# zhangganlin/GlORIE-SLAM

Measured on AMD Instinct MI355X. Metric: DSPO BA-update iters/sec + rendered rays/sec, 640x480 Replica keyframe graph, higher is better.
Workload: dtype f16 corr/ConvGRU, f32 Jacobians, f64 solve; render: f32 (decoder matmuls as 3-term f16 splits, f32 accumulate); 1 GPU; G8: 8 keyframes, 36 edges, 60x80 (640x480/8), BA itrs=2, DSPO stages alternating, context part of the GRU gates (one map per source keyframe) re-evaluated for all keyframes every 12 steps; multiview_filter.thresh = 0.25 (reference ships 0.01, configs/mono_point_slam.yaml:75: with untrained weights 0.01 rejects > 80 % of every frame and no depth_scale step would reach stage 2); render: 524k-point c; edges_local=36, edges_total=36, hw=4800, keyframes=8, parallelism=single GPU

## Files before the change

glorie_slam_amd/csrc/ba.hip:

```cpp
#include <hip/hip_runtime.h>
#include <stdint.h>
#include <math.h>
#include "common.hiph"
#include "se3.hiph"
#include "ba_common.hiph"

namespace glorie {

__device__ __forceinline__ void block_inclusive_scan(int* a, int n) {
  const int tid = threadIdx.x;
  for (int off = 1; off < n; off <<= 1) {
    int tmp[4];
#pragma unroll
    for (int q = 0; q < 4; ++q) {
      const int f = tid + q * 1024;
      tmp[q] = (f < n) ? a[f] + (f >= off ? a[f - off] : 0) : 0;
    }
    __syncthreads();
#pragma unroll
    for (int q = 0; q < 4; ++q) {
      const int f = tid + q * 1024;
      if (f < n) a[f] = tmp[q];
    }
    __syncthreads();
  }
}

__global__ __launch_bounds__(1024) void ba_prepare_kernel(BaWork wk, const int64_t* __restrict__ ii,
                                                          int B, int N, int M, int t0, int t1) {
  if (ba_skipped(wk)) return;
  extern __shared__ int sm[];
  int* cnt = sm;
  int* scan = sm + B;
  int* slot = sm + 2 * B;
  int* eii = sm + 3 * B;
  const int tid = threadIdx.x;
  if (tid == 0 && wk.gate_hits) atomicAdd(wk.gate_hits, 1);
  for (int f = tid; f < B; f += 1024) cnt[f] = 0;
  if (tid < 4) wk.status[tid] = 0;
  __syncthreads();
  for (int n = tid; n < N; n += 1024) {
    const int f = (int)ii[n];
    eii[n] = f;
    if (f >= 0 && f < B) atomicAdd(&cnt[f], 1);
  }
  __syncthreads();
  for (int f = tid; f < B; f += 1024) scan[f] = (cnt[f] > 0 || (f >= t0 && f < t1)) ? 1 : 0;
  __syncthreads();
  block_inclusive_scan(scan, B);
  const int Mdev = B > 0 ? scan[B - 1] : 0;
  for (int f = tid; f < B; f += 1024) {
    const int present = (cnt[f] > 0 || (f >= t0 && f < t1)) ? 1 : 0;
    const int sl = present ? scan[f] - 1 : -1;
    slot[f] = sl;
    wk.slot_of_frame[f] = sl;
    if (sl >= 0 && sl < M) wk.kx[sl] = f;
  }
  if (tid == 0) {
    wk.status[1] = Mdev;
    if (Mdev != M) atomicOr(&wk.status[0], BA_ST_M_MISMATCH);
  }
  __syncthreads();
  if (Mdev != M) return;
  for (int sl = tid; sl < M; sl += 1024) scan[sl] = 0;
  __syncthreads();
  for (int f = tid; f < B; f += 1024)
    if (slot[f] >= 0) scan[slot[f]] = cnt[f];
  __syncthreads();
  block_inclusive_scan(scan, M);
  for (int sl = tid; sl <= M; sl += 1024) wk.csr_ptr[sl] = (sl == 0) ? 0 : scan[sl - 1];
  for (int f = tid; f < B; f += 1024) {
    const int sl = slot[f];
    if (sl < 0 || cnt[f] == 0) continue;
    int o = (sl == 0) ? 0 : scan[sl - 1];
    for (int n = 0; n < N; ++n)
      if (eii[n] == f) wk.csr_edge[o++] = n;
  }
}

struct PixJ {
  float Ju[6], Jv[6];
  float Jzu, Jzv;
  float ru, rv;
  float wu, wv;
};

__device__ __forceinline__ void pixel_terms(const Pose g, float fx, float fy, float cx, float cy,
                                            float u, float v, float disp, float tu, float tv,
                                            float wgt_u, float wgt_v, PixJ& o) {
  float Xi[4], Xj[4];
  Xi[0] = (u - cx) / fx;
  Xi[1] = (v - cy) / fy;
  Xi[2] = 1.0f;
  Xi[3] = disp;
  se3_act(g, Xi, Xj);
  const float x = Xj[0], y = Xj[1], hh = Xj[3];
  const bool near = Xj[2] < 0.25f;
  const float d = near ? 0.0f : 1.0f / Xj[2];
  const float d2 = d * d;
  o.wu = near ? 0.0f : 0.001f * wgt_u;
  o.wv = near ? 0.0f : 0.001f * wgt_v;
  o.ru = tu - (fx * d * x + cx);
  o.rv = tv - (fy * d * y + cy);
  o.Ju[0] = fx * (hh * d);
  o.Ju[1] = fx * 0.0f;
  o.Ju[2] = fx * (-x * hh * d2);
  o.Ju[3] = fx * (-x * y * d2);
  o.Ju[4] = fx * (1.0f + x * x * d2);
  o.Ju[5] = fx * (-y * d);
  o.Jzu = fx * (g.t.x * d - g.t.z * (x * d2));
  o.Jv[0] = fy * 0.0f;
  o.Jv[1] = fy * (hh * d);
  o.Jv[2] = fy * (-y * hh * d2);
  o.Jv[3] = fy * (-1.0f - y * y * d2);
  o.Jv[4] = fy * (x * y * d2);
  o.Jv[5] = fy * (x * d);
  o.Jzv = fy * (g.t.y * d - g.t.z * (y * d2));
}

__device__ __forceinline__ void edge_adjoint(const Pose g, float L[36]) {
#pragma unroll
  for (int m = 0; m < 6; ++m) {
    float X[6] = {0, 0, 0, 0, 0, 0}, Y[6];
    X[m] = 1.0f;
    se3_adjT(g, X, Y);
#pragma unroll
    for (int r = 0; r < 6; ++r) L[r * 6 + m] = Y[r];
  }
}

// ... 548 lines not shown
      hr[q] = Bj[ok[q] ? o_ar[q] - 1 : 0];
      hc[q] = Bj[ok[q] ? o_ac[q] - 1 : 0];
      cur[q] = Bj[ok[q] ? o_w[q] : 0];
      if (!inr) ar[q] = 0.0;
      if (!inc) ac[q] = 0.0;
    }
    const bool rok = j + 1 + rhs_dc < n, rin = rok && rhs_dc < bw;
    double ra = Bj[rin ? o_rc : 0];
    const double rh = Bj[rok ? o_rc - 1 : 0];
    const double ru = u[rok ? j + 1 + rhs_dc : 0];
    const double u0 = u[j], u1h = u[j + 1];
    if (!rin) ra = 0.0;
    const double ri0 = rcp_f64(d0);
    const double d1 = h11 - a1 * ri0 * a1;
    if ((!(d0 > 0.0) || !(d1 > 0.0)) && tid == 0) *fail = 1;
    const double ri1 = rcp_f64(d1);
    if (tid == 0) { rinv[j] = ri0; rinv[j + 1] = ri1; }
#pragma unroll
    for (int q = 0; q < NQ; ++q) {
      if (pend_on[q]) B[(j - 2) * S + o_w[q]] = pend[q];
      pend_on[q] = false;
      if (!ok[q]) continue;
      double v = cur[q] - ar[q] * ri0 * ac[q];
      if (e_dc[q] > 0) {
        const double br = hr[q] - ar[q] * ri0 * a1, bc = hc[q] - ac[q] * ri0 * a1;
        v -= br * ri1 * bc;
        B[j * S + o_w[q]] = v;
      } else {
        pend[q] = v;
        pend_on[q] = true;
      }
    }
    if (rok) {
      double v = ru - u0 * ri0 * ra;
      if (rhs_dc > 0) {
        const double u1 = u1h - u0 * ri0 * a1, bc = rh - ra * ri0 * a1;
        v -= u1 * ri1 * bc;
      }
      u[j + 1 + rhs_dc] = v;
    }
    __syncthreads();
  }
#pragma unroll
  for (int q = 0; q < NQ; ++q)
    if (pend_on[q]) B[(j - 2) * S + o_w[q]] = pend[q];
  if (j < n) {
    const double d = B[j * S];
    if (!(d > 0.0) && tid == 0) *fail = 1;
    if (tid == 0) rinv[j] = rcp_f64(d);
  }
  __syncthreads();
}

__global__ __launch_bounds__(kBandThreads) void ba_solve_band_kernel(BaWork wk, int n, float lm, float ep,
                                                                    int lds_doubles, int force_bw, int from_acc) {
  if (ba_skipped(wk)) return;
  extern __shared__ double bsm[];
  __shared__ int fail, bw_s;
  const int tid = threadIdx.x;
  const double* A = wk.Hd;
  if (tid == 0) {
    fail = (wk.status[0] & (BA_ST_M_MISMATCH | BA_ST_NONFINITE)) ? 1 : 0;
    bw_s = force_bw >= 0 ? force_bw : wk.status[3] >> 1;
  }
  __syncthreads();
  const int bw = bw_s;
  const int S = bw + 1;
  if (bw >= 64 || (size_t)n * S + 2 * (size_t)n > (size_t)lds_doubles) {
    return;
  }
  double* B = bsm;
  double* u = B + (size_t)n * S;
  double* rinv = u + n;
  for (int base = tid; base < n * S; base += kBandThreads * 8) {
    double v[8];
    int rr[8], kk[8];
#pragma unroll
    for (int q = 0; q < 8; ++q) {
      const int idx = base + q * kBandThreads;
      const int r = idx / S, k = S - 1 - (idx - r * S);
      rr[q] = r; kk[q] = k;
      v[q] = (idx < n * S && k <= r) ? (from_acc ? acc_value(wk.Hacc, (size_t)r * n + r - k) : A[(size_t)r * n + r - k]) : 0.0;
    }
#pragma unroll
    for (int q = 0; q < 8; ++q) {
      if (base + q * kBandThreads >= n * S) continue;
      double x = v[q];
      if (kk[q] == 0) x += (double)ep + (double)lm * x;
      B[rr[q] * S + kk[q]] = x;
    }
  }
  for (int i = tid; i < n; i += kBandThreads)
    u[i] = from_acc ? acc_value(wk.Hacc, (size_t)n * n + i) : A[(size_t)n * n + i];
  if ((bw + 1) * (bw + 2) / 2 <= 4 * kBandThreads) band_eliminate<4>(B, u, rinv, &fail, n, bw);
  else band_eliminate<9>(B, u, rinv, &fail, n, bw);
  if (fail) {
    for (int i = tid; i < n; i += kBandThreads) wk.dx[i] = 0.0f;
    if (tid == 0) {
      atomicOr(&wk.status[0], BA_ST_CHOL_FAILED);
      atomicAdd(&wk.status[2], 1);
      if (force_bw < 0) wk.status[3] = (bw << 1) | 1;
    }
    return;
  }
  if (tid < 64) {
    double srow = 0.0;
    double un = u[n - 1], rn = rinv[n - 1];
    int dn = (n - 1 - tid) & 63;
    double bn = B[(n - 1) * S + min(dn, bw)];
    for (int j = n - 1; j >= 0; --j) {
      const double uc = un, rc = rn, bc = bn;
      const int dist = dn;
      if (j > 0) {
        un = u[j - 1]; rn = rinv[j - 1];
        dn = (j - 1 - tid) & 63;
        bn = B[(j - 1) * S + min(dn, bw)];
      }
      const int lo = j & 63;
      const double xj_own = (uc - srow) * rc;
      const unsigned lo32 = __builtin_amdgcn_readlane((int)__double2loint(xj_own), lo);
      const unsigned hi32 = __builtin_amdgcn_readlane((int)__double2hiint(xj_own), lo);
      const double xj = __hiloint2double((int)hi32, (int)lo32);
      if (tid == lo) { srow = 0.0; wk.dx[j] = (float)xj; }
      if (dist >= 1 && dist <= bw && j - dist >= 0) srow = fma(bc, xj, srow);
    }
  }
  if (tid == 0 && force_bw < 0) wk.status[3] = (bw << 1) | 1;
}

constexpr int kCB = 32;
constexpr int kCBP = kCB + 1;
constexpr int kFusedMaxN = 540;

__global__ __launch_bounds__(1024) void ba_solve_fused_kernel(BaWork wk, int n, float lm, float ep) {
  if (ba_skipped(wk)) return;
  extern __shared__ double fsm[];
  double* Dl = fsm;
  double* Wl = Dl + kCB * kCBP;
  double* P = Wl + kCB * kCBP;
  __shared__ int fail, bw_s;
  const int tid = threadIdx.x;
  double* A = wk.Hd;
  if (tid == 0) { fail = (wk.status[0] & (BA_ST_M_MISMATCH | BA_ST_NONFINITE)) ? 1 : 0; bw_s = wk.status[3]; }
  __syncthreads();
  if (tid == 0) wk.status[3] = 0;
  if (bw_s & 1) return;
  for (int i = tid; i < n; i += 1024) {
    const double v = A[(size_t)i * n + i];
    A[(size_t)i * n + i] = v + (double)ep + (double)lm * v;
  }
  __syncthreads();
  const int bw = bw_s >> 1;
  const int br = tid >> 5, bc = tid & 31;
  for (int j0 = 0; j0 < n; j0 += kCB) {
    const int nb = min(kCB, n - j0);
    const int rem = min(n - j0 - nb, bw);
    const int base = j0 + nb;
    if (br < nb && bc <= br) {
      Dl[br * kCBP + bc] = A[(size_t)(j0 + br) * n + j0 + bc];
      Wl[br * kCBP + bc] = br == bc ? 1.0 : 0.0;
    }
    __syncthreads();
    for (int j = 0; j < nb; ++j) {
      const double d = Dl[j * kCBP + j];
      if (!(d > 0.0) && tid == 0) fail = 1;
      if (br < nb && br > j) {
        const double mlt = Dl[br * kCBP + j] / d;
        if (bc > j && bc <= br) Dl[br * kCBP + bc] -= mlt * Dl[bc * kCBP + j];
        else if (bc <= j) Wl[br * kCBP + bc] -= mlt * Wl[j * kCBP + bc];
      }
      __syncthreads();
    }
    double lval = 0.0, wval = 0.0;
    if (br < nb && bc <= br) {
      const double sc = sqrt(Dl[bc * kCBP + bc]), sr = sqrt(Dl[br * kCBP + br]);
      lval = (br == bc) ? sc : Dl[br * kCBP + bc] / sc;
      wval = Wl[br * kCBP + bc] / sr;
    }
    __syncthreads();
// ... 180 lines not shown
  const double* ap = P + tl * kCBP;
#pragma unroll 4
  for (int m = 0; m < kCB; ++m) {
    const double am = ap[m];
#pragma unroll
    for (int q = 0; q < 4; ++q) x[q] = fma(am, (m <= 8 * q + g) ? wg[8 * q * kCBP + m] : 0.0, x[q]);
  }
  if (t <= rem) {
    double* arow = A + (size_t)(t < rem ? base + t : n) * n + j0;
#pragma unroll
    for (int q = 0; q < 4; ++q) {
      const int c = 8 * q + g;
      if (c < nb) arow[c] = x[q];
    }
  }
}

__global__ __launch_bounds__(256) void chol_backsub_block_kernel(BaWork wk, int n, int j0, int nb) {
  if (ba_skipped(wk)) return;
  __shared__ double Wl[kCB * kCBP], yb[kCB], xb[kCB];
  const int tid = threadIdx.x;
  double* A = wk.Hd;
  double* y = A + (size_t)n * n;
  if (wk.status[0] & (BA_ST_SOLVE_ABORT | BA_ST_M_MISMATCH)) {
    if (blockIdx.x == 0 && tid < nb) wk.dx[j0 + tid] = 0.0f;
    return;
  }
  for (int idx = tid; idx < kCB * kCB; idx += 256) {
    const int r = idx >> 5, c = idx & 31;
    double v = 0.0;
    if (r < nb && c < nb) {
      if (c < r) v = A[(size_t)(j0 + c) * n + j0 + r];
      else if (c == r) v = 1.0 / A[(size_t)(j0 + r) * n + j0 + r];
    }
    Wl[r * kCBP + c] = v;
  }
  if (tid < kCB) yb[tid] = tid < nb ? y[j0 + tid] : 0.0;
  __syncthreads();
  if (tid < kCB) {
    double v = 0.0;
    for (int r = tid; r < nb; ++r) v = fma(Wl[r * kCBP + tid], yb[r], v);
    xb[tid] = v;
  }
  __syncthreads();
  if (blockIdx.x == 0 && tid < nb) wk.dx[j0 + tid] = (float)xb[tid];
  const int r = blockIdx.x * 256 + tid;
  if (r < j0) {
    double v = y[r];
    for (int c = 0; c < nb; ++c) v -= A[(size_t)(j0 + c) * n + r] * xb[c];
    y[r] = v;
  }
}

__global__ __launch_bounds__(kBaThreads) void ba_update_kernel(
    BaWork wk, float* __restrict__ poses, float* __restrict__ disps,
    const int64_t* __restrict__ ii, const int64_t* __restrict__ jj, int HW, int t0, int t1,
    int motion_only, int depth_only, float* __restrict__ dx_out, float* __restrict__ dz_out) {
  if (ba_skipped(wk)) return;
  constexpr int EB = 128;
  __shared__ float ys[EB * 6];
  const int tid = threadIdx.x;
  const int s = blockIdx.y;
  if (wk.status[0] & BA_ST_M_MISMATCH) return;
  const int P = t1 - t0;
  if (blockIdx.x == 0 && s == 0) {
    for (int p = tid; p < P; p += kBaThreads) {
      float xi[6];
#pragma unroll
      for (int q = 0; q < 6; ++q) xi[q] = wk.dx[p * 6 + q];
      if (dx_out) {
#pragma unroll
        for (int q = 0; q < 6; ++q) dx_out[p * 6 + q] = xi[q];
      }
      if (!depth_only) {
        float* pp = poses + (size_t)(t0 + p) * 7;
        const Pose g = se3_retract(xi, load_pose(pp));
        pp[0] = g.t.x; pp[1] = g.t.y; pp[2] = g.t.z;
        pp[3] = g.q.x; pp[4] = g.q.y; pp[5] = g.q.z; pp[6] = g.q.w;
      }
    }
  }
  if (motion_only) return;
  const int k = wk.kx[s];
  const int e0 = wk.csr_ptr[s];
  const int deg = wk.csr_ptr[s + 1] - e0;
  const int pk = k - t0;
  const bool self_on = (pk > 0 && pk < P);
  const int px = blockIdx.x * kBaThreads + tid;
  float dw = 0.0f;
  for (int a0 = 0; a0 < deg; a0 += EB) {
    const int nb = min(EB, deg - a0);
    __syncthreads();
    for (int idx = tid; idx < nb * 6; idx += kBaThreads) {
      const int a = idx / 6, r = idx % 6;
      const int n = wk.csr_edge[e0 + a0 + a];
      const int pj = (int)jj[n] - t0;
      float y = (pj > 0 && pj < P) ? wk.dx[pj * 6 + r] : 0.0f;
      if (self_on) {
        const float* L = wk.Ledge + (size_t)n * 36;
        float acc = 0.0f;
#pragma unroll
        for (int m = 0; m < 6; ++m) acc += L[m * 6 + r] * wk.dx[pk * 6 + m];
        y -= acc;
      }
      ys[idx] = y;
    }
    __syncthreads();
    if (px < HW) {
      for (int a = 0; a < nb; ++a) {
        const int n = wk.csr_edge[e0 + a0 + a];
#pragma unroll
        for (int r = 0; r < 6; ++r) dw += wk.Eij[((size_t)n * 6 + r) * HW + px] * ys[a * 6 + r];
      }
    }
  }
  if (px >= HW) return;
  const float dz = wk.Q[(size_t)s * HW + px] * (wk.W[(size_t)s * HW + px] - dw);
  disps[(size_t)k * HW + px] += dz;
  if (dz_out) dz_out[(size_t)s * HW + px] = dz;
}

int ba_prepare(const BaWork& wk, const int64_t* ii, int B, int N, int M, int t0, int t1,
               hipStream_t st) {
  const size_t prep_lds = sizeof(int) * ((size_t)3 * B + (size_t)N);
  if (prep_lds > 150 * 1024) return GLORIE_EUNSUPPORTED;
  static PerDeviceOnce attr_set;
  if (attr_set.first()) {
    (void)hipFuncSetAttribute(reinterpret_cast<const void*>(ba_prepare_kernel),
                              hipFuncAttributeMaxDynamicSharedMemorySize, 150 * 1024);
  }
  hipLaunchKernelGGL(ba_prepare_kernel, dim3(1), dim3(1024), prep_lds, st, wk, ii, B, N, M, t0, t1);
  return check_launch();
}

}

using namespace glorie;

namespace glorie {

struct BaPlan {
  BaWork wk;
  int B, N, M, h, w, HW, t0, t1, P, n6, ppt, chunk_px, nchunks;
  size_t scratch_used;
};

static int ba_plan(glorie_ctx* ctx, int B, int N, int M, int h, int w, int t0, int t1,
                   double* hv_ext, BaPlan& pl) {
  if (!ctx || B < 0 || N < 0 || M < 0 || h < 0 || w < 0 || t1 < t0) return GLORIE_EINVAL;
  if (B > kMaxFramesLds || N > kMaxEdgesLds || t1 > B) return GLORIE_EUNSUPPORTED;
  pl.B = B; pl.N = N; pl.M = M; pl.h = h; pl.w = w; pl.HW = h * w; pl.t0 = t0; pl.t1 = t1;
  pl.P = t1 - t0; pl.n6 = 6 * pl.P;
#ifdef EXP_BA_CHUNK_WGS
  constexpr long kChunkWgs = EXP_BA_CHUNK_WGS;
#else
// ... 25 lines not shown
  pl.scratch_used = off;
  char* base = reinterpret_cast<char*>(ctx->scratch);
  BaWork& wk = pl.wk;
  wk.slot_of_frame = reinterpret_cast<int*>(base + o_slot);
  wk.kx = reinterpret_cast<int*>(base + o_kx);
  wk.csr_ptr = reinterpret_cast<int*>(base + o_ptr);
  wk.csr_edge = reinterpret_cast<int*>(base + o_edge);
  wk.status = ctx->dstatus;
  wk.Ledge = reinterpret_cast<float*>(base + o_L);
  wk.Eij = reinterpret_cast<float*>(base + o_E);
  wk.Hpart = reinterpret_cast<float*>(base + o_Hp);
  wk.Q = reinterpret_cast<float*>(base + o_Q);
  wk.W = reinterpret_cast<float*>(base + o_W);
  wk.CWpart = reinterpret_cast<float*>(base + o_CW);
  wk.Hd = hv_ext ? hv_ext : reinterpret_cast<double*>(base + o_Hd);
  wk.vd = wk.Hd + n6 * n6;
  wk.Hacc = reinterpret_cast<unsigned long long*>(base + o_acc);
  wk.dx = reinterpret_cast<float*>(base + o_dx);
  wk.gate = ctx->ba_gate;
  wk.gate_hits = nullptr;
  static PerDeviceOnce attr_set;
  if (attr_set.first()) {
    (void)hipFuncSetAttribute(reinterpret_cast<const void*>(ba_solve_fused_kernel),
                              hipFuncAttributeMaxDynamicSharedMemorySize, 160 * 1024 - 64);
    (void)hipFuncSetAttribute(reinterpret_cast<const void*>(ba_solve_band_kernel),
                              hipFuncAttributeMaxDynamicSharedMemorySize, 160 * 1024 - 64);
  }
  return GLORIE_OK;
}

static int ba_build_system(const BaPlan& pl, const float* poses, const float* disps,
                           const float* intrinsics, const float* disps_sens, const float* targets,
                           const float* weights, const float* eta, const int64_t* ii,
                           const int64_t* jj, int flags, bool to_f64, hipStream_t st) {
  const BaWork& wk = pl.wk;
  const int motion_only = flags & 1, hwc = (flags & GLORIE_BA_TARGETS_HWC) ? 1 : 0;
  hipLaunchKernelGGL(ba_jacobian_kernel, dim3(pl.nchunks, pl.N), dim3(kBaThreads), 0, st, wk, poses,
                     disps, intrinsics, disps_sens, targets, weights, eta, ii, jj, pl.HW, pl.w,
                     pl.nchunks, pl.ppt, motion_only, hwc, (long)pl.n6 * pl.n6 + pl.n6);
  if (!motion_only)
    hipLaunchKernelGGL(ba_gram_kernel, dim3(pl.nchunks, pl.M), dim3(kBaThreads), 0, st, wk, ii, jj, pl.HW,
                       pl.chunk_px, pl.t0, pl.t1, pl.nchunks, eta, disps, disps_sens);
  else
    hipLaunchKernelGGL(ba_assemble_kernel, dim3(pl.N), dim3(64), 0, st, wk, ii, jj, pl.nchunks, pl.t0, pl.t1);
  if (to_f64) {
    const long total = (long)pl.n6 * pl.n6 + pl.n6;
    hipLaunchKernelGGL(ba_system_f64_kernel, dim3((unsigned)((total + 255) / 256)), dim3(256), 0, st, wk, total);
  }
  return check_launch();
}

static int ba_solve_update(const BaPlan& pl, float* poses, float* disps, const int64_t* ii,
                           const int64_t* jj, float lm, float ep, int motion_only, int depth_only,
                           float* dx_out, float* dz_out, bool from_acc, hipStream_t st) {
  const BaWork& wk = pl.wk;
  const int n6 = pl.n6;
  if (n6 <= kSolveMaxN) {
    const int bwf = n6 > 1 ? n6 - 1 : 1;
    const int need = n6 * (bwf + 1) + 2 * n6;
    hipLaunchKernelGGL(ba_solve_band_kernel, dim3(1), dim3(kBandThreads), sizeof(double) * (size_t)need, st, wk, n6,
                       lm, ep, need, bwf, from_acc ? 1 : 0);
  } else if (n6 <= kFusedMaxN) {
    const size_t rows = (size_t)(n6 + 1 > kCB ? n6 + 1 - kCB : 1);
    const size_t lds = sizeof(double) * (2 * kCB * kCBP + (rows * kCBP > (size_t)n6 ? rows * kCBP : (size_t)n6));
    const int band_doubles = (160 * 1024 - 256) / (int)sizeof(double);
    hipLaunchKernelGGL(ba_bandwidth_kernel, dim3(n6), dim3(64), 0, st, wk, n6);
    hipLaunchKernelGGL(ba_solve_band_kernel, dim3(1), dim3(kBandThreads), sizeof(double) * (size_t)band_doubles, st,
                       wk, n6, lm, ep, band_doubles, -1, 0);
    hipLaunchKernelGGL(ba_solve_fused_kernel, dim3(1), dim3(1024), lds, st, wk, n6, lm, ep);
  } else {
    hipLaunchKernelGGL(chol_damp_kernel, dim3((n6 + 255) / 256), dim3(256), 0, st, wk, n6, lm, ep);
    for (int j0 = 0; j0 < n6; j0 += kCB) {
      const int nb = (n6 - j0 < kCB) ? (n6 - j0) : kCB;
      const int rem = n6 - j0 - nb;
      hipLaunchKernelGGL(chol_diag_inv_kernel, dim3(1), dim3(1024), 0, st, wk, n6, j0, nb);
      hipLaunchKernelGGL(chol_panel_gemm_kernel, dim3((rem + kPanelRows) / kPanelRows), dim3(1024), 0, st, wk, n6, j0, nb);
      if (rem > 0) {
        const int tl = (rem + kTrailTile) / kTrailTile;
        hipLaunchKernelGGL(chol_trail_kernel, dim3(tl, tl), dim3(256), 0, st, wk, n6, j0, nb);
      }
    }
    for (int j0 = ((n6 - 1) / kCB) * kCB; j0 >= 0; j0 -= kCB) {
      const int nb = (n6 - j0 < kCB) ? (n6 - j0) : kCB;
      hipLaunchKernelGGL(chol_backsub_block_kernel, dim3(j0 > 0 ? (j0 + 255) / 256 : 1), dim3(256), 0, st, wk, n6, j0,
                         nb);
    }
  }
  const int upd_chunks = (pl.HW + kBaThreads - 1) / kBaThreads;
  hipLaunchKernelGGL(ba_update_kernel, dim3(upd_chunks, pl.M), dim3(kBaThreads), 0, st, wk, poses,
                     disps, ii, jj, pl.HW, pl.t0, pl.t1, motion_only, depth_only, dx_out, dz_out);
  return check_launch();
}

__global__ __launch_bounds__(256) void ba_zero_gated_kernel(const int* __restrict__ gate, int* __restrict__ dstatus,
                                                            double* __restrict__ hv, size_t n) {
  if (*gate != 0) return;
  const size_t i = (size_t)blockIdx.x * 256 + threadIdx.x;
  if (i < 4) dstatus[i] = 0;
  if (i < n) hv[i] = 0.0;
}

}

extern "C" int glorie_ba(glorie_ctx* ctx, float* poses, float* disps, const float* intrinsics,
                         const float* disps_sens, const float* targets, const float* weights,
                         const float* eta, const int64_t* ii, const int64_t* jj, int B, int N,
                         int M, int h, int w, int t0, int t1, int iterations, float lm, float ep,
                         int motion_only, int depth_only, float* dx_out, float* dz_out,
                         void* stream) {
  if (iterations < 0) return GLORIE_EINVAL;
  const int flags = motion_only;
  motion_only = flags & 1;
  BaPlan pl;
  GLORIE_TRY(ba_plan(ctx, B, N, M, h, w, t0, t1, nullptr, pl));
  if (N == 0 || pl.P == 0 || pl.HW == 0 || iterations == 0) return GLORIE_OK;
  if (!poses || !disps || !intrinsics || !targets || !weights || !ii || !jj) return GLORIE_EINVAL;
  if (!motion_only && !eta) return GLORIE_EINVAL;
  hipStream_t st = (hipStream_t)stream;
  GLORIE_TRY(ctx_poison(ctx, pl.scratch_used, st));
  {
    BaWork w0 = pl.wk;
    if (ctx->ba_gate && ctx->ba_gate_count) { w0.gate_hits = ctx->ba_gate_hits; ctx->ba_gate_count = false; }
    GLORIE_TRY(ba_prepare(w0, ii, B, N, M, t0, t1, st));
  }
  const bool direct = pl.n6 <= kSolveMaxN;
  for (int it = 0; it < iterations; ++it) {
    GLORIE_TRY(ba_build_system(pl, poses, disps, intrinsics, disps_sens, targets, weights, eta, ii, jj,
                               flags, !direct, st));
    GLORIE_TRY(ba_solve_update(pl, poses, disps, ii, jj, lm, ep, motion_only, depth_only, dx_out,
                               dz_out, direct, st));
  }
  return GLORIE_OK;
}

extern "C" int glorie_ba_build_system(glorie_ctx* ctx, const float* poses, const float* disps,
                                      const float* intrinsics, const float* disps_sens,
                                      const float* targets, const float* weights, const float* eta,
                                      const int64_t* ii, const int64_t* jj, int B, int N, int M,
                                      int h, int w, int t0, int t1, int motion_only, double* hv_out,
                                      void* stream) {
  BaPlan pl;
  GLORIE_TRY(ba_plan(ctx, B, N, M, h, w, t0, t1, hv_out, pl));
  if (!hv_out || pl.P == 0) return GLORIE_EINVAL;
  hipStream_t st = (hipStream_t)stream;
  if (N == 0 || pl.HW == 0) {
    const size_t nhv = (size_t)pl.n6 * pl.n6 + pl.n6;
    if (ctx->ba_gate) {
      hipLaunchKernelGGL(ba_zero_gated_kernel, dim3((unsigned)((nhv + 255) / 256)), dim3(256), 0, st, ctx->ba_gate,
                         ctx->dstatus, hv_out, nhv);
      return check_launch();
    }
    GLORIE_TRY(check_hip(hipMemsetAsync(ctx->dstatus, 0, 4 * sizeof(int), st)));
    return check_hip(hipMemsetAsync(hv_out, 0, sizeof(double) * nhv, st));
  }
  if (!poses || !disps || !intrinsics || !targets || !weights || !ii || !jj) return GLORIE_EINVAL;
  if (!(motion_only & 1) && !eta) return GLORIE_EINVAL;
  GLORIE_TRY(ctx_poison(ctx, pl.scratch_used, st));
  {
    BaWork w0 = pl.wk;
    if (ctx->ba_gate && ctx->ba_gate_count) { w0.gate_hits = ctx->ba_gate_hits; ctx->ba_gate_count = false; }
    GLORIE_TRY(ba_prepare(w0, ii, B, N, M, t0, t1, st));
  }
  return ba_build_system(pl, poses, disps, intrinsics, disps_sens, targets, weights, eta, ii, jj,
                         motion_only, true, st);
}

extern "C" int glorie_ba_solve_update(glorie_ctx* ctx, float* poses, float* disps,
                                      const int64_t* ii, const int64_t* jj, int B, int N, int M,
                                      int h, int w, int t0, int t1, float lm, float ep,
                                      int motion_only, int depth_only, const double* hv,
                                      float* dx_out, float* dz_out, void* stream) {
  BaPlan pl;
  GLORIE_TRY(ba_plan(ctx, B, N, M, h, w, t0, t1, const_cast<double*>(hv), pl));
  if (!hv || !poses || !disps || pl.P == 0) return GLORIE_EINVAL;
  if (N > 0 && (!ii || !jj)) return GLORIE_EINVAL;
  hipStream_t st = (hipStream_t)stream;
  if (N == 0 || pl.HW == 0) {
    pl.M = 1;
    return ba_solve_update(pl, poses, disps, ii, jj, lm, ep, 1, depth_only, dx_out,
                           nullptr, false, st);
  }
  return ba_solve_update(pl, poses, disps, ii, jj, lm, ep, motion_only, depth_only, dx_out, dz_out,
                         false, st);
// ... 45 lines not shown
```

glorie_slam_amd/csrc/dspo.hip:

```cpp
#include <hip/hip_runtime.h>
#include <stdint.h>
#include "common.hiph"
#include "se3.hiph"
#include "ba_common.hiph"

namespace glorie {

struct Dspo2Args {
  const float* poses;
  float* disps;
  const float* intr;
  const float* mono;
  float* scales;
  float* shifts;
  const uint8_t* vmask;
  const float* target;
  const float* weight;
  const float* eta;
  const int64_t* ii;
  const int64_t* jj;
  const uint8_t* edge_on;
  float alpha;
};

// ... 7 lines not shown
  j.Js = invalid ? 0.0f : -mono * sa;
  j.Jq = invalid ? 0.0f : -sa;
  return j;
}

__device__ __forceinline__ bool frame_enabled(const BaWork& wk, const uint8_t* edge_on, int s) {
  if (!edge_on) return wk.csr_ptr[s + 1] > wk.csr_ptr[s];
  for (int ei = wk.csr_ptr[s]; ei < wk.csr_ptr[s + 1]; ++ei)
    if (edge_on[wk.csr_edge[ei]]) return true;
  return false;
}

__global__ __launch_bounds__(256) void dspo2_solve_kernel(BaWork wk, Dspo2Args a, int M, int nchunks,
                                                          float lm, float ep) {
  __shared__ int fail;
  const int tid = threadIdx.x;
  if (tid == 0) fail = 0;
  __syncthreads();
  if (wk.status[0] & BA_ST_M_MISMATCH) return;
  for (int s = tid; s < M; s += 256) {
    const bool on = frame_enabled(wk, a.edge_on, s);
    double x1 = 0.0, x2 = 0.0;
    if (on) {
      double v[10];
      for (int q = 0; q < 10; ++q) v[q] = 0.0;
      for (int c = 0; c < nchunks; ++c)
        for (int q = 0; q < 10; ++q) v[q] += (double)wk.Hpart[((size_t)s * nchunks + c) * 10 + q];
      const double H11 = v[0] + ep + lm * v[0], H22 = v[2] + ep + lm * v[2];
      const double S11 = H11 - v[3], S12 = v[1] - v[4], S22 = H22 - v[5];
      const double b1 = v[6] - v[8], b2 = v[7] - v[9];
      const double l21 = (S11 > 0.0) ? S12 / sqrt(S11) : 0.0;
      const double l22sq = S22 - l21 * l21;
      if (!(S11 > 0.0) || !(l22sq > 0.0)) {
        atomicOr(&fail, 1);
      } else {
        const double det = S11 * S22 - S12 * S12;
        x1 = (S22 * b1 - S12 * b2) / det;
        x2 = (S11 * b2 - S12 * b1) / det;
      }
    }
    wk.dx[2 * s + 0] = (float)x1;
    wk.dx[2 * s + 1] = (float)x2;
  }
  __syncthreads();
  if (fail) {
    for (int s = tid; s < 2 * M; s += 256) wk.dx[s] = 0.0f;
    if (tid == 0) {
      atomicOr(&wk.status[0], BA_ST_CHOL_FAILED);
      atomicAdd(&wk.status[2], 1);
    }
  }
}

__global__ __launch_bounds__(kBaThreads) void dspo2_accum_kernel(BaWork wk, Dspo2Args a, int HW,
                                                                 int w, int nchunks) {
  __shared__ float red[4][10];
  const int tid = threadIdx.x, lane = tid & 63, wv = tid >> 6;
  const int chunk = blockIdx.x, s = blockIdx.y;
  if (wk.status[0] & BA_ST_M_MISMATCH) return;
  const int k = wk.kx[s];
  const int e0 = wk.csr_ptr[s], e1 = wk.csr_ptr[s + 1];
  const int px = chunk * kBaThreads + tid;
  const bool live = px < HW;
  float Cp = 0.0f, Wp = 0.0f;
  int n_on = 0;
  const float fxi = a.intr[k * 4 + 0], fyi = a.intr[k * 4 + 1];
  const float cxi = a.intr[k * 4 + 2], cyi = a.intr[k * 4 + 3];
  const int yy = live ? px / w : 0, xx = live ? px - yy * w : 0;
  const float dsp = live ? a.disps[(size_t)k * HW + px] : 1.0f;
  for (int ei = e0; ei < e1; ++ei) {
    const int n = wk.csr_edge[ei];
    if (a.edge_on && !a.edge_on[n]) continue;
    ++n_on;
    const int jx = (int)a.jj[n];
    const Pose g = (jx == k) ? stereo_pose()
                             : relative_pose(load_pose(a.poses + k * 7), load_pose(a.poses + jx * 7));
    const float fxj = a.intr[jx * 4 + 0], fyj = a.intr[jx * 4 + 1];
    const float cxj = a.intr[jx * 4 + 2], cyj = a.intr[jx * 4 + 3];
    if (!live) continue;
    float X0[4], X1[4];
    X0[0] = ((float)xx - cxi) / fxi;
    X0[1] = ((float)yy - cyi) / fyi;
    X0[2] = 1.0f;
    X0[3] = dsp;
    se3_act(g, X0, X1);
    const float Z = (X1[2] < 0.1f) ? 1.0f : X1[2];
    const float d = 1.0f / Z;
    const float cu = fxj * (X1[0] * d) + cxj, cv = fyj * (X1[1] * d) + cyj;
    const float valid = (X1[2] > 0.2f) ? 1.0f : 0.0f;
    const float2 tg = reinterpret_cast<const float2*>(a.target)[(size_t)n * HW + px];
    const float2 wg = reinterpret_cast<const float2*>(a.weight)[(size_t)n * HW + px];
    const float wu = 0.001f * (valid * wg.x), wvv = 0.001f * (valid * wg.y);
    const float ru = tg.x - cu, rv = tg.y - cv;
    const float Jzu = fxj * d * g.t.x - fxj * X1[0] * d * d * g.t.z;
    const float Jzv = fyj * d * g.t.y - fyj * X1[1] * d * d * g.t.z;
    Cp += wu * Jzu * Jzu + wvv * Jzv * Jzv;
    Wp += wu * ru * Jzu + wvv * rv * Jzv;
  }
  if (n_on != 0) {
    float sums[10];
#pragma unroll
    for (int q = 0; q < 10; ++q) sums[q] = 0.0f;
    if (live) {
      const float mono = a.mono[(size_t)k * HW + px];
      const PriorJ J = prior_jacobians(mono, a.vmask[(size_t)k * HW + px] != 0, a.alpha);
      const float rd = sqrtf(a.alpha) * (dsp - (a.scales[k] * mono + a.shifts[k]));
      const float C = Cp + J.Jd * J.Jd + a.eta[(size_t)s * HW + px];
      const float Wv = Wp - J.Jd * rd;
      const float Q = 1.0f / C;
      wk.Q[(size_t)s * HW + px] = Q;
      wk.W[(size_t)s * HW + px] = Wv;
      const float e1v = J.Js * J.Jd, e2v = J.Jq * J.Jd;
      sums[0] = J.Js * J.Js; sums[1] = J.Js * J.Jq; sums[2] = J.Jq * J.Jq;
      sums[3] = e1v * Q * e1v; sums[4] = e1v * Q * e2v; sums[5] = e2v * Q * e2v;
      sums[6] = -J.Js * rd; sums[7] = -J.Jq * rd;
      sums[8] = e1v * Q * Wv; sums[9] = e2v * Q * Wv;
    }
#pragma unroll
    for (int q = 0; q < 10; ++q) sums[q] = wave_sum(sums[q]);
    if (lane == 0) {
#pragma unroll
      for (int q = 0; q < 10; ++q) red[wv][q] = sums[q];
    }
    __syncthreads();
// ... 66 lines not shown
  }
  const int px = blockIdx.x * kBaThreads + tid;
  if (px >= HW) return;
  const PriorJ J = prior_jacobians(a.mono[(size_t)k * HW + px], a.vmask[(size_t)k * HW + px] != 0, a.alpha);
  const float dz = wk.Q[(size_t)s * HW + px] *
                   (wk.W[(size_t)s * HW + px] - (J.Js * J.Jd * ds + J.Jq * J.Jd * dq));
  a.disps[(size_t)k * HW + px] = fmaxf(a.disps[(size_t)k * HW + px] + dz, 0.0f);
  if (dz_out) dz_out[(size_t)s * HW + px] = dz;
}

}

using namespace glorie;

extern "C" int glorie_dspo_scale_shift(glorie_ctx* ctx, const float* poses, float* disps,
                                       const float* intrinsics, const float* mono_disps,
                                       float* scales, float* shifts, const uint8_t* valid_mask,
                                       const float* target, const float* weight, const float* eta,
                                       const int64_t* ii, const int64_t* jj, const uint8_t* edge_on,
                                       int B, int N, int M, int h, int w, int iterations, float lm,
                                       float ep, float alpha, float* dz_out, void* stream) {
  if (!ctx || B < 0 || N < 0 || M < 0 || h < 0 || w < 0 || iterations < 0) return GLORIE_EINVAL;
  const int HW = h * w;
  if (N == 0 || M == 0 || HW == 0 || iterations == 0) return GLORIE_OK;
  if (!poses || !disps || !intrinsics || !mono_disps || !scales || !shifts || !valid_mask || !target ||
      !weight || !eta || !ii || !jj)
    return GLORIE_EINVAL;
  if (B > kMaxFramesLds || N > kMaxEdgesLds) return GLORIE_EUNSUPPORTED;
  hipStream_t st = (hipStream_t)stream;
  const int nchunks = (HW + kBaThreads - 1) / kBaThreads;
  size_t off = 0;
  auto carve = [&](size_t bytes) { size_t o = off; off = align_up(off + bytes, 256); return o; };
  const size_t o_slot = carve(sizeof(int) * (size_t)B);
  const size_t o_kx = carve(sizeof(int) * (size_t)(M + 1));
  const size_t o_ptr = carve(sizeof(int) * (size_t)(M + 2));
  const size_t o_edge = carve(sizeof(int) * (size_t)N);
  const size_t o_Hp = carve(sizeof(float) * 10 * (size_t)M * nchunks);
  const size_t o_Q = carve(sizeof(float) * (size_t)M * HW);
  const size_t o_W = carve(sizeof(float) * (size_t)M * HW);
  const size_t o_dx = carve(sizeof(float) * 2 * (size_t)M);
  GLORIE_TRY(ctx_reserve(ctx, off));
  GLORIE_TRY(ctx_poison(ctx, off, st));
  char* base = reinterpret_cast<char*>(ctx->scratch);
  BaWork wk{};
  wk.slot_of_frame = reinterpret_cast<int*>(base + o_slot);
  wk.kx = reinterpret_cast<int*>(base + o_kx);
  wk.csr_ptr = reinterpret_cast<int*>(base + o_ptr);
  wk.csr_edge = reinterpret_cast<int*>(base + o_edge);
  wk.status = ctx->dstatus;
  wk.Hpart = reinterpret_cast<float*>(base + o_Hp);
  wk.Q = reinterpret_cast<float*>(base + o_Q);
  wk.W = reinterpret_cast<float*>(base + o_W);
  wk.dx = reinterpret_cast<float*>(base + o_dx);
  GLORIE_TRY(ba_prepare(wk, ii, B, N, M, 0, 0, st));
  Dspo2Args a{poses, disps, intrinsics, mono_disps, scales, shifts, valid_mask, target, weight, eta,
              ii, jj, edge_on, alpha};
  for (int it = 0; it < iterations; ++it) {
    hipLaunchKernelGGL(dspo2_accum_kernel, dim3(nchunks, M), dim3(kBaThreads), 0, st, wk, a, HW, w, nchunks);
    if (M <= 25) {
      hipLaunchKernelGGL(dspo2_update_kernel<true>, dim3(nchunks, M), dim3(kBaThreads), 0, st, wk, a, HW, dz_out, M,
                         nchunks, lm, ep);
    } else {
      hipLaunchKernelGGL(dspo2_solve_kernel, dim3(1), dim3(256), 0, st, wk, a, M, nchunks, lm, ep);
      hipLaunchKernelGGL(dspo2_update_kernel<false>, dim3(nchunks, M), dim3(kBaThreads), 0, st, wk, a, HW, dz_out, M,
                         nchunks, lm, ep);
    }
    GLORIE_TRY(check_launch());
  }
  return GLORIE_OK;
}
```

Baseline: 962.9 BA-update iters/s.

## Fold band solve into BA update launch and prep tables into first DSPO accum

New measurement: 964.2 BA-update iters/s, median of 6. Within noise of the previous version (+0.1%).

```diff
diff --git a/glorie_slam_amd/csrc/ba.hip b/glorie_slam_amd/csrc/ba.hip
--- a/glorie_slam_amd/csrc/ba.hip
+++ b/glorie_slam_amd/csrc/ba.hip
@@ -7,75 +7,11 @@
 
 namespace glorie {
 
-__device__ __forceinline__ void block_inclusive_scan(int* a, int n) {
-  const int tid = threadIdx.x;
-  for (int off = 1; off < n; off <<= 1) {
-    int tmp[4];
-#pragma unroll
-    for (int q = 0; q < 4; ++q) {
-      const int f = tid + q * 1024;
-      tmp[q] = (f < n) ? a[f] + (f >= off ? a[f - off] : 0) : 0;
-    }
-    __syncthreads();
-#pragma unroll
-    for (int q = 0; q < 4; ++q) {
-      const int f = tid + q * 1024;
-      if (f < n) a[f] = tmp[q];
-    }
-    __syncthreads();
-  }
-}
-
 __global__ __launch_bounds__(1024) void ba_prepare_kernel(BaWork wk, const int64_t* __restrict__ ii,
                                                           int B, int N, int M, int t0, int t1) {
   if (ba_skipped(wk)) return;
   extern __shared__ int sm[];
-  int* cnt = sm;
-  int* scan = sm + B;
-  int* slot = sm + 2 * B;
-  int* eii = sm + 3 * B;
-  const int tid = threadIdx.x;
-  if (tid == 0 && wk.gate_hits) atomicAdd(wk.gate_hits, 1);
-  for (int f = tid; f < B; f += 1024) cnt[f] = 0;
-  if (tid < 4) wk.status[tid] = 0;
-  __syncthreads();
-  for (int n = tid; n < N; n += 1024) {
-    const int f = (int)ii[n];
-    eii[n] = f;
-    if (f >= 0 && f < B) atomicAdd(&cnt[f], 1);
-  }
-  __syncthreads();
-  for (int f = tid; f < B; f += 1024) scan[f] = (cnt[f] > 0 || (f >= t0 && f < t1)) ? 1 : 0;
-  __syncthreads();
-  block_inclusive_scan(scan, B);
-  const int Mdev = B > 0 ? scan[B - 1] : 0;
-  for (int f = tid; f < B; f += 1024) {
-    const int present = (cnt[f] > 0 || (f >= t0 && f < t1)) ? 1 : 0;
-    const int sl = present ? scan[f] - 1 : -1;
-    slot[f] = sl;
-    wk.slot_of_frame[f] = sl;
-    if (sl >= 0 && sl < M) wk.kx[sl] = f;
-  }
-  if (tid == 0) {
-    wk.status[1] = Mdev;
-    if (Mdev != M) atomicOr(&wk.status[0], BA_ST_M_MISMATCH);
-  }
-  __syncthreads();
-  if (Mdev != M) return;
-  for (int sl = tid; sl < M; sl += 1024) scan[sl] = 0;
-  __syncthreads();
-  for (int f = tid; f < B; f += 1024)
-    if (slot[f] >= 0) scan[slot[f]] = cnt[f];
-  __syncthreads();
-  block_inclusive_scan(scan, M);
-  for (int sl = tid; sl <= M; sl += 1024) wk.csr_ptr[sl] = (sl == 0) ? 0 : scan[sl - 1];
-  for (int f = tid; f < B; f += 1024) {
-    const int sl = slot[f];
-    if (sl < 0 || cnt[f] == 0) continue;
-    int o = (sl == 0) ? 0 : scan[sl - 1];
-    for (int n = 0; n < N; ++n)
-      if (eii[n] == f) wk.csr_edge[o++] = n;
-  }
+  ba_prepare_tables<1024>(wk, ii, B, N, M, t0, t1, sm);
 }
 
 struct PixJ {
@@ -730,26 +666,11 @@
   __syncthreads();
 }
 
-__global__ __launch_bounds__(kBandThreads) void ba_solve_band_kernel(BaWork wk, int n, float lm, float ep,
-                                                                    int lds_doubles, int force_bw, int from_acc) {
-  if (ba_skipped(wk)) return;
-  extern __shared__ double bsm[];
-  __shared__ int fail, bw_s;
+__device__ __forceinline__ void band_load_eliminate(const BaWork& wk, const double* __restrict__ A, int n, float lm,
+                                                    float ep, int bw, int from_acc, double* B, double* u, double* rinv,
+                                                    int* fail) {
   const int tid = threadIdx.x;
-  const double* A = wk.Hd;
-  if (tid == 0) {
-    fail = (wk.status[0] & (BA_ST_M_MISMATCH | BA_ST_NONFINITE)) ? 1 : 0;
-    bw_s = force_bw >= 0 ? force_bw : wk.status[3] >> 1;
-  }
-  __syncthreads();
-  const int bw = bw_s;
   const int S = bw + 1;
-  if (bw >= 64 || (size_t)n * S + 2 * (size_t)n > (size_t)lds_doubles) {
-    return;
-  }
-  double* B = bsm;
-  double* u = B + (size_t)n * S;
-  double* rinv = u + n;
   for (int base = tid; base < n * S; base += kBandThreads * 8) {
     double v[8];
     int rr[8], kk[8];
@@ -770,17 +691,14 @@
   }
   for (int i = tid; i < n; i += kBandThreads)
     u[i] = from_acc ? acc_value(wk.Hacc, (size_t)n * n + i) : A[(size_t)n * n + i];
-  if ((bw + 1) * (bw + 2) / 2 <= 4 * kBandThreads) band_eliminate<4>(B, u, rinv, &fail, n, bw);
-  else band_eliminate<9>(B, u, rinv, &fail, n, bw);
-  if (fail) {
-    for (int i = tid; i < n; i += kBandThreads) wk.dx[i] = 0.0f;
-    if (tid == 0) {
-      atomicOr(&wk.status[0], BA_ST_CHOL_FAILED);
-      atomicAdd(&wk.status[2], 1);
-      if (force_bw < 0) wk.status[3] = (bw << 1) | 1;
-    }
-    return;
-  }
+  if ((bw + 1) * (bw + 2) / 2 <= 4 * kBandThreads) band_eliminate<4>(B, u, rinv, fail, n, bw);
+  else band_eliminate<9>(B, u, rinv, fail, n, bw);
+}
+
+__device__ __forceinline__ void band_back_substitute(const double* B, const double* u, const double* rinv, int n, int bw,
+                                                     float* dx) {
+  const int tid = threadIdx.x;
+  const int S = bw + 1;
   if (tid < 64) {
     double srow = 0.0;
     double un = u[n - 1], rn = rinv[n - 1];
@@ -799,10 +717,43 @@
       const unsigned lo32 = __builtin_amdgcn_readlane((int)__double2loint(xj_own), lo);
       const unsigned hi32 = __builtin_amdgcn_readlane((int)__double2hiint(xj_own), lo);
       const double xj = __hiloint2double((int)hi32, (int)lo32);
-      if (tid == lo) { srow = 0.0; wk.dx[j] = (float)xj; }
+      if (tid == lo) { srow = 0.0; dx[j] = (float)xj; }
       if (dist >= 1 && dist <= bw && j - dist >= 0) srow = fma(bc, xj, srow);
     }
   }
+}
+
+__global__ __launch_bounds__(kBandThreads) void ba_solve_band_kernel(BaWork wk, int n, float lm, float ep,
+                                                                    int lds_doubles, int force_bw, int from_acc) {
+  if (ba_skipped(wk)) return;
+  extern __shared__ double bsm[];
+  __shared__ int fail, bw_s;
+  const int tid = threadIdx.x;
+  const double* A = wk.Hd;
+  if (tid == 0) {
+    fail = (wk.status[0] & (BA_ST_M_MISMATCH | BA_ST_NONFINITE)) ? 1 : 0;
+    bw_s = force_bw >= 0 ? force_bw : wk.status[3] >> 1;
+  }
+  __syncthreads();
+  const int bw = bw_s;
+  const int S = bw + 1;
+  if (bw >= 64 || (size_t)n * S + 2 * (size_t)n > (size_t)lds_doubles) {
+    return;
+  }
+  double* B = bsm;
+  double* u = B + (size_t)n * S;
+  double* rinv = u + n;
+  band_load_eliminate(wk, A, n, lm, ep, bw, from_acc, B, u, rinv, &fail);
+  if (fail) {
+    for (int i = tid; i < n; i += kBandThreads) wk.dx[i] = 0.0f;
+    if (tid == 0) {
+      atomicOr(&wk.status[0], BA_ST_CHOL_FAILED);
+      atomicAdd(&wk.status[2], 1);
+      if (force_bw < 0) wk.status[3] = (bw << 1) | 1;
+    }
+    return;
+  }
+  band_back_substitute(B, u, rinv, n, bw, wk.dx);
   if (tid == 0 && force_bw < 0) wk.status[3] = (bw << 1) | 1;
 }
 
@@ -1089,22 +1040,66 @@
   }
 }
 
+template <bool SOLVE>
 __global__ __launch_bounds__(kBaThreads) void ba_update_kernel(
     BaWork wk, float* __restrict__ poses, float* __restrict__ disps,
     const int64_t* __restrict__ ii, const int64_t* __restrict__ jj, int HW, int t0, int t1,
-    int motion_only, int depth_only, float* __restrict__ dx_out, float* __restrict__ dz_out) {
+    int motion_only, int depth_only, float* __restrict__ dx_out, float* __restrict__ dz_out, float lm, float ep) {
   if (ba_skipped(wk)) return;
+  static_assert(kBaThreads == kBandThreads, "the band solve runs in the update launch's workgroups");
   constexpr int EB = 128;
   __shared__ float ys[EB * 6];
+  __shared__ float sdx[SOLVE ? kSolveMaxN : 1];
+  __shared__ int fail;
   const int tid = threadIdx.x;
   const int s = blockIdx.y;
-  if (wk.status[0] & BA_ST_M_MISMATCH) return;
   const int P = t1 - t0;
-  if (blockIdx.x == 0 && s == 0) {
+  const bool first = blockIdx.x == 0 && s == 0;
+  if (wk.status[0] & BA_ST_M_MISMATCH) {
+    if constexpr (SOLVE) {
+      if (first) {
+        for (int i = tid; i < 6 * P; i += kBaThreads) wk.dx[i] = 0.0f;
+        if (tid == 0) {
+          atomicOr(&wk.status[0], BA_ST_CHOL_FAILED);
+          atomicAdd(&wk.status[2], 1);
+        }
+      }
+    }
+    return;
+  }
+  if constexpr (SOLVE) {
+    if (motion_only && !first) return;
+    extern __shared__ double bsm[];
+    const int n = 6 * P, bw = n > 1 ? n - 1 : 1;
+    double* B = bsm;
+    double* u = B + (size_t)n * (bw + 1);
+    double* rinv = u + n;
+    if (tid == 0) fail = (wk.status[0] & BA_ST_NONFINITE) ? 1 : 0;
+    __syncthreads();
+    band_load_eliminate(wk, nullptr, n, lm, ep, bw, 1, B, u, rinv, &fail);
+    if (fail) {
+      for (int i = tid; i < n; i += kBaThreads) sdx[i] = 0.0f;
+    } else {
+      band_back_substitute(B, u, rinv, n, bw, sdx);
+    }
+    __syncthreads();
+    if (first) {
+      for (int i = tid; i < n; i += kBaThreads) wk.dx[i] = sdx[i];
+      if (fail && tid == 0) {
+        atomicOr(&wk.status[0], BA_ST_CHOL_FAILED);
+        atomicAdd(&wk.status[2], 1);
+      }
+    }
+  }
+  auto dxv = [&](int i) -> float {
+    if constexpr (SOLVE) return sdx[i];
+    else return wk.dx[i];
+  };
+  if (first) {
     for (int p = tid; p < P; p += kBaThreads) {
       float xi[6];
 #pragma unroll
-      for (int q = 0; q < 6; ++q) xi[q] = wk.dx[p * 6 + q];
+      for (int q = 0; q < 6; ++q) xi[q] = dxv(p * 6 + q);
       if (dx_out) {
 #pragma unroll
         for (int q = 0; q < 6; ++q) dx_out[p * 6 + q] = xi[q];
@@ -1132,12 +1127,12 @@
       const int a = idx / 6, r = idx % 6;
       const int n = wk.csr_edge[e0 + a0 + a];
       const int pj = (int)jj[n] - t0;
-      float y = (pj > 0 && pj < P) ? wk.dx[pj * 6 + r] : 0.0f;
+      float y = (pj > 0 && pj < P) ? dxv(pj * 6 + r) : 0.0f;
       if (self_on) {
         const float* L = wk.Ledge + (size_t)n * 36;
         float acc = 0.0f;
 #pragma unroll
-        for (int m = 0; m < 6; ++m) acc += L[m * 6 + r] * wk.dx[pk * 6 + m];
+        for (int m = 0; m < 6; ++m) acc += L[m * 6 + r] * dxv(pk * 6 + m);
         y -= acc;
       }
       ys[idx] = y;
@@ -1269,9 +1264,18 @@
 
 static int ba_solve_update(const BaPlan& pl, float* poses, float* disps, const int64_t* ii,
                            const int64_t* jj, float lm, float ep, int motion_only, int depth_only,
-                           float* dx_out, float* dz_out, bool from_acc, hipStream_t st) {
+                           float* dx_out, float* dz_out, bool from_acc, hipStream_t st,
+                           bool solve_in_update = false) {
   const BaWork& wk = pl.wk;
   const int n6 = pl.n6;
+  const int upd_chunks = (pl.HW + kBaThreads - 1) / kBaThreads;
+  if (solve_in_update) {
+    const int bwf = n6 > 1 ? n6 - 1 : 1;
+    const int need = n6 * (bwf + 1) + 2 * n6;
+    hipLaunchKernelGGL(ba_update_kernel<true>, dim3(upd_chunks, pl.M), dim3(kBaThreads), sizeof(double) * (size_t)need,
+                       st, wk, poses, disps, ii, jj, pl.HW, pl.t0, pl.t1, motion_only, depth_only, dx_out, dz_out, lm, ep);
+    return check_launch();
+  }
   if (n6 <= kSolveMaxN) {
     const int bwf = n6 > 1 ? n6 - 1 : 1;
     const int need = n6 * (bwf + 1) + 2 * n6;
@@ -1303,9 +1307,8 @@
                          nb);
     }
   }
-  const int upd_chunks = (pl.HW + kBaThreads - 1) / kBaThreads;
-  hipLaunchKernelGGL(ba_update_kernel, dim3(upd_chunks, pl.M), dim3(kBaThreads), 0, st, wk, poses,
-                     disps, ii, jj, pl.HW, pl.t0, pl.t1, motion_only, depth_only, dx_out, dz_out);
+  hipLaunchKernelGGL(ba_update_kernel<false>, dim3(upd_chunks, pl.M), dim3(kBaThreads), 0, st, wk, poses,
+                     disps, ii, jj, pl.HW, pl.t0, pl.t1, motion_only, depth_only, dx_out, dz_out, lm, ep);
   return check_launch();
 }
 
@@ -1341,11 +1344,13 @@
     GLORIE_TRY(ba_prepare(w0, ii, B, N, M, t0, t1, st));
   }
   const bool direct = pl.n6 <= kSolveMaxN;
+  const bool solve_in_update = direct && (long)((pl.HW + kBaThreads - 1) / kBaThreads) * M <= kChainMaxUpdateWgs &&
+                               !solver_chain_legacy();
   for (int it = 0; it < iterations; ++it) {
     GLORIE_TRY(ba_build_system(pl, poses, disps, intrinsics, disps_sens, targets, weights, eta, ii, jj,
                                flags, !direct, st));
     GLORIE_TRY(ba_solve_update(pl, poses, disps, ii, jj, lm, ep, motion_only, depth_only, dx_out,
-                               dz_out, direct, st));
+                               dz_out, direct, st, solve_in_update));
   }
   return GLORIE_OK;
 }
diff --git a/glorie_slam_amd/csrc/dspo.hip b/glorie_slam_amd/csrc/dspo.hip
--- a/glorie_slam_amd/csrc/dspo.hip
+++ b/glorie_slam_amd/csrc/dspo.hip
@@ -83,14 +83,59 @@
   }
 }
 
+template <bool PREP>
 __global__ __launch_bounds__(kBaThreads) void dspo2_accum_kernel(BaWork wk, Dspo2Args a, int HW,
-                                                                 int w, int nchunks) {
+                                                                 int w, int nchunks, int B, int N, int M) {
   __shared__ float red[4][10];
+  __shared__ unsigned long long present[PREP ? kChainMaxFrames / 64 : 1];
+  __shared__ int elist[PREP ? kChainMaxEdges : 1];
+  __shared__ int wcnt[4];
   const int tid = threadIdx.x, lane = tid & 63, wv = tid >> 6;
   const int chunk = blockIdx.x, s = blockIdx.y;
-  if (wk.status[0] & BA_ST_M_MISMATCH) return;
-  const int k = wk.kx[s];
-  const int e0 = wk.csr_ptr[s], e1 = wk.csr_ptr[s + 1];
+  int k, e0, e1;
+  if constexpr (PREP) {
+    static_assert(kChainMaxEdges <= kBaThreads, "one edge per thread");
+    extern __shared__ int prep_sm[];
+    if (s == M) {
+      if (chunk == 0) ba_prepare_tables<kBaThreads>(wk, a.ii, B, N, M, 0, 0, prep_sm);
+      return;
+    }
+    if (tid < kChainMaxFrames / 64) present[tid] = 0ull;
+    __syncthreads();
+    int f = -1;
+    if (tid < N) {
+      f = (int)a.ii[tid];
+      if (f >= 0 && f < B) atomicOr(&present[f >> 6], 1ull << (f & 63));
+      else f = -1;
+    }
+    __syncthreads();
+    int Mdev = 0;
+    k = -1;
+    for (int q = 0; q < kChainMaxFrames / 64; ++q) {
+      unsigned long long m = present[q];
+      const int c = __popcll(m);
+      if (k < 0 && s < Mdev + c) {
+        for (int r = s - Mdev; r > 0; --r) m &= m - 1;
+        k = q * 64 + __ffsll((long long)m) - 1;
+      }
+      Mdev += c;
+    }
+    if (Mdev != M) return;
+    const unsigned long long mine = __ballot(f == k);
+    if (lane == 0) wcnt[wv] = __popcll(mine);
+    __syncthreads();
+    int off = 0;
+    for (int q = 0; q < wv; ++q) off += wcnt[q];
+    if (f == k) elist[off + __popcll(mine & ((1ull << lane) - 1ull))] = tid;
+    e0 = 0;
+    e1 = wcnt[0] + wcnt[1] + wcnt[2] + wcnt[3];
+    __syncthreads();
+  } else {
+    if (wk.status[0] & BA_ST_M_MISMATCH) return;
+    k = wk.kx[s];
+    e0 = wk.csr_ptr[s];
+    e1 = wk.csr_ptr[s + 1];
+  }
   const int px = chunk * kBaThreads + tid;
   const bool live = px < HW;
   float Cp = 0.0f, Wp = 0.0f;
@@ -100,7 +145,9 @@
   const int yy = live ? px / w : 0, xx = live ? px - yy * w : 0;
   const float dsp = live ? a.disps[(size_t)k * HW + px] : 1.0f;
   for (int ei = e0; ei < e1; ++ei) {
-    const int n = wk.csr_edge[ei];
+    int n;
+    if constexpr (PREP) n = elist[ei];
+    else n = wk.csr_edge[ei];
     if (a.edge_on && !a.edge_on[n]) continue;
     ++n_on;
     const int jx = (int)a.jj[n];
@@ -273,11 +320,17 @@
   wk.Q = reinterpret_cast<float*>(base + o_Q);
   wk.W = reinterpret_cast<float*>(base + o_W);
   wk.dx = reinterpret_cast<float*>(base + o_dx);
-  GLORIE_TRY(ba_prepare(wk, ii, B, N, M, 0, 0, st));
+  const bool chain = M <= 25 && B <= kChainMaxFrames && N <= kChainMaxEdges && !solver_chain_legacy();
+  if (!chain) GLORIE_TRY(ba_prepare(wk, ii, B, N, M, 0, 0, st));
   Dspo2Args a{poses, disps, intrinsics, mono_disps, scales, shifts, valid_mask, target, weight, eta,
               ii, jj, edge_on, alpha};
   for (int it = 0; it < iterations; ++it) {
-    hipLaunchKernelGGL(dspo2_accum_kernel, dim3(nchunks, M), dim3(kBaThreads), 0, st, wk, a, HW, w, nchunks);
+    if (chain && it == 0)
+      hipLaunchKernelGGL(dspo2_accum_kernel<true>, dim3(nchunks, M + 1), dim3(kBaThreads),
+                         sizeof(int) * ((size_t)3 * B + (size_t)N), st, wk, a, HW, w, nchunks, B, N, M);
+    else
+      hipLaunchKernelGGL(dspo2_accum_kernel<false>, dim3(nchunks, M), dim3(kBaThreads), 0, st, wk, a, HW, w, nchunks, B,
+                         N, M);
     if (M <= 25) {
       hipLaunchKernelGGL(dspo2_update_kernel<true>, dim3(nchunks, M), dim3(kBaThreads), 0, st, wk, a, HW, dz_out, M,
                          nchunks, lm, ep);
```
